# openpsi-project/srl

Measured on NVIDIA B200. Metric: gae_ppo_loss_transitions_per_sec, higher is better.
Workload: dtype f32

## Files before the change

### include/srl_b200.h

```cpp
#ifndef SRL_B200_H_
#define SRL_B200_H_

#include <stddef.h>
#include <stdint.h>

#ifdef __cplusplus
extern "C" {
#endif

#define SRL_B200_ABI_VERSION 12

typedef void* srl_stream_t;

enum srl_status {
  SRL_OK = 0,
  SRL_ERR_INVALID_ARG = 1,
  SRL_ERR_UNSUPPORTED = 2,
  SRL_ERR_CUDA = 3,
  SRL_ERR_NO_DEVICE = 4
};

const char* srl_last_error(void);
int srl_abi_version(void);
int srl_pdl_enabled(void);
int srl_set_pdl(int on);
int srl_device_info(int* sm_count, int* cc_major, int* cc_minor);

#define SRL_LANE_PART 8

int srl_gae_scan(const float* reward,
                 const float* value,
                 const uint8_t* done,
                 const uint8_t* truncated,
                 const uint8_t* on_reset,
                 const float* vtrace_new_logp,
                 const float* vtrace_old_logp,
                 const double* popart_mean_std,
                 const float* old_logp,
                 int L, int N, int row_lo, int row_hi, double gamma, double lmbda, double rho, double c,
                 float* adv,
                 float* ret,
                 double* lane_part,
                 double* lane_aos,
                 float* pack,
                 srl_stream_t stream);

int srl_gae_scan_perm(const float* reward, const float* value, const uint8_t* done, const uint8_t* truncated,
                      const uint8_t* on_reset, const float* vtrace_new_logp, const float* vtrace_old_logp,
                      const double* popart_mean_std, const float* old_logp, int L, int N, int row_lo, int row_hi,
                      double gamma, double lmbda, double rho, double c, float* adv, float* ret, double* lane_part,
                      double* lane_aos, float* pack, uint64_t perm_seed, uint32_t perm_epoch, int perm_n_epochs,
                      int perm_n_env, int perm_group, int32_t* perm_out, int perm_minibatches, double* minibatch_part,
                      int* fused, srl_stream_t stream);

int srl_gae_trace(const float* reward,
                  const float* value,
                  const uint8_t* done,
                  const uint8_t* truncated,
                  const uint8_t* on_reset,
                  const float* gamma_t,
                  const float* lmbda_t,
                  const float* imp_ratio,
                  int L, int N, int critic_dim, double gamma, double lmbda, double rho, double c, int pad_last_row,
                  float* adv, float* ret, srl_stream_t stream);

int srl_traj_gae(const void* reward, const void* value, const int64_t* offsets ,
                 const uint8_t* final_truncated ,
                 const uint8_t* final_has_value , int n_traj, int width, int is_float64,
                 double gamma, double lmbda, void* adv, void* ret, srl_stream_t stream);

int srl_n_step_return(const float* reward, const float* nex_value, const uint8_t* nex_done,
                      const uint8_t* nex_truncated, int n, int rows, int N, double gamma, float* out,
                      srl_stream_t stream);

int srl_lane_stats(const float* adv, const float* ret, const uint8_t* done, const uint8_t* truncated,
                   const uint8_t* on_reset, int L, int N, int row_lo, int row_hi, double* lane_part,
                   srl_stream_t stream);

size_t srl_group_stats_workspace_bytes(int G, int whole_first);
int srl_group_stats(const double* lane_part, int N, const int32_t* idx, int G, int per, int whole_first,
                    double* out, void* workspace, size_t workspace_bytes, srl_stream_t stream);

int srl_popart_update(const double* batch_stats, double* state, double beta, double eps, double* mean_std_out,
                      srl_stream_t stream);

enum srl_value_loss { SRL_VL_MSE = 0, SRL_VL_HUBER = 1, SRL_VL_SMOOTHL1 = 2 };

// ... 184 lines not shown
```

### srl_b200/_lib.py

```python
from __future__ import annotations

import ctypes
import os
from ctypes import POINTER, c_char_p, c_double, c_int, c_int32, c_int64, c_size_t, c_uint32, c_uint64, c_void_p

_HERE = os.path.dirname(os.path.abspath(__file__))
_LIB_NAME = "libsrl_b200.so"

SRL_LANE_PART = 8
SRL_LOSS_OUT_LEN = 16
SRL_MAX_LEAVES = 32
SRL_MAX_HEADS = 8
SRL_K4B_MAX_SUM_K = 199
SRL_K4B_MAX_SUM_K_MASKED = 159
SRL_MAX_LOSS_BATCH = 32
ABI_VERSION = 12

OUT_LOSS, OUT_POLICY_LOSS, OUT_VALUE_LOSS, OUT_ENTROPY_LOSS = 0, 1, 2, 3
OUT_ADVANTAGE, OUT_IMPORTANCE_WEIGHT, OUT_CLIP_RATIO, OUT_VALUE_TARGETS, OUT_DENORM_VALUE, OUT_MASK_SUM = 4, 5, 6, 7, 8, 9
VALUE_LOSS_CODES = {"mse": 0, "huber": 1, "smoothl1": 2}


class MissingCudaLibrary(RuntimeError):
    """libsrl_b200.so has not been built; run `python -m srl_b200.build` (needs nvcc)."""


class SrlCudaError(RuntimeError):

    def __init__(self, fn: str, status: int, message: str):
        super().__init__(f"{fn} failed with status {status}: {message}")
        self.fn, self.status, self.message = fn, status, message


class PpoHyper(ctypes.Structure):
    _fields_ = [
        ("eps_clip", c_double),
        ("value_eps_clip", c_double),
        ("c_clip", c_double),
        ("value_loss_weight", c_double),
        ("entropy_bonus_weight", c_double),
        ("vl_param", c_double),
        ("adv_eps", c_double),
        ("value_loss", c_int32),
        ("clip_value", c_int32),
        ("dual_clip", c_int32),
        ("normalize_old_value", c_int32),
    ]


class LossProblem(ctypes.Structure):
    _fields_ = [(k, c_void_p) for k in ("new_logp", "v_pred", "entropy", "lane_idx", "norm_stats", "local_stats",
                                        "g_logp", "g_value", "g_entropy", "out", "out_f32", "workspace")]


class LeafDesc(ctypes.Structure):
    _fields_ = [("src", c_void_p), ("dst", c_void_p), ("row_bytes", c_int64), ("src_slots", c_int64),
                ("src_t_stride", c_int64), ("src_slot_stride", c_int64)]


SIGNATURES = {
    "srl_last_error": (c_char_p, []),
    "srl_abi_version": (c_int, []),
    "srl_pdl_enabled": (c_int, []),
    "srl_set_pdl": (c_int, [c_int]),
    "srl_device_info": (c_int, [POINTER(c_int), POINTER(c_int), POINTER(c_int)]),
    "srl_gae_scan": (c_int, [c_void_p] * 9 + [c_int, c_int, c_int, c_int, c_double, c_double, c_double, c_double] +
                     [c_void_p, c_void_p, c_void_p, c_void_p, c_void_p, c_void_p]),
    "srl_gae_scan_perm": (c_int, [c_void_p] * 9 + [c_int, c_int, c_int, c_int, c_double, c_double, c_double, c_double] +
                          [c_void_p, c_void_p, c_void_p, c_void_p, c_void_p] +
                          [ctypes.c_uint64, ctypes.c_uint32, c_int, c_int, c_int, c_void_p, c_int, c_void_p, c_void_p,
                           c_void_p]),
    "srl_gae_trace": (c_int, [c_void_p] * 8 + [c_int, c_int, c_int, c_double, c_double, c_double, c_double, c_int,
                              c_void_p, c_void_p, c_void_p]),
    "srl_traj_gae": (c_int, [c_void_p] * 5 + [c_int, c_int, c_int, c_double, c_double, c_void_p, c_void_p, c_void_p]),
    "srl_n_step_return": (c_int, [c_void_p] * 4 + [c_int, c_int, c_int, c_double, c_void_p, c_void_p]),
    "srl_lane_stats": (c_int, [c_void_p] * 5 + [c_int, c_int, c_int, c_int, c_void_p, c_void_p]),
    "srl_group_stats_workspace_bytes": (c_size_t, [c_int, c_int]),
    "srl_group_stats": (c_int, [c_void_p, c_int, c_void_p, c_int, c_int, c_int, c_void_p, c_void_p, c_size_t, c_void_p]),
    "srl_popart_update": (c_int, [c_void_p, c_void_p, c_double, c_double, c_void_p, c_void_p]),
    "srl_ppo_loss_workspace_bytes": (c_size_t, [c_int, c_int]),
    "srl_ppo_loss_finalize": (c_int, [c_void_p, c_size_t, c_int, c_void_p, c_void_p, c_void_p]),
    "srl_ppo_loss_fwd_bwd": (c_int, [c_void_p, c_void_p, c_void_p, c_int64,
                                     c_void_p, c_void_p, c_void_p, c_void_p, c_void_p, c_int64, c_void_p,
                                     c_int, c_int, c_void_p, c_void_p, c_void_p, POINTER(PpoHyper),
                                     c_void_p, c_void_p, c_void_p, c_int64, c_void_p, c_void_p, c_void_p, c_size_t,
                                     c_void_p]),
    "srl_ppo_loss_fwd_bwd_batched": (c_int, [POINTER(LossProblem), c_int, c_int64, c_int64,
                                             c_void_p, c_void_p, c_void_p, c_void_p, c_void_p, c_int64, c_void_p,
                                             c_int, c_void_p, c_void_p, c_int, c_int, c_int, c_int, c_void_p, POINTER(PpoHyper),
                                             c_size_t, c_void_p, c_void_p]),
    "srl_ppo_loss_from_logits": (c_int, [c_void_p, c_void_p, POINTER(c_int32), c_int, c_void_p,
                                         c_void_p, c_void_p, c_void_p, c_void_p, c_void_p, c_int64, c_void_p,
                                         c_int, c_int, c_void_p, c_void_p, c_void_p, POINTER(PpoHyper),
                                         c_void_p, c_void_p, c_void_p, c_void_p, c_void_p, c_void_p, c_void_p,
                                         c_size_t, c_void_p]),
    "srl_ppo_loss_from_logits_masked": (c_int, [c_void_p, c_void_p, c_void_p, POINTER(c_int32), c_int, c_void_p,
                                                c_void_p, c_void_p, c_void_p, c_void_p, c_void_p, c_int64, c_void_p,
                                                c_int, c_int, c_void_p, c_void_p, c_void_p, POINTER(PpoHyper),
                                                c_void_p, c_void_p, c_void_p, c_void_p, c_void_p, c_void_p, c_void_p,
                                                c_size_t, c_void_p]),
    "srl_ppo_loss_from_logits_bf16": (c_int, [c_void_p, c_void_p, POINTER(c_int32), c_int, c_void_p,
                                              c_void_p, c_void_p, c_void_p, c_void_p, c_void_p, c_int64, c_void_p,
                                              c_int, c_int, c_void_p, c_void_p, c_void_p, POINTER(PpoHyper),
                                              c_void_p, c_void_p, c_void_p, c_void_p, c_void_p, c_void_p, c_void_p,
# ... 106 lines not shown
```

### srl_b200/csrc/gae_common.cuh

```cuda
#pragma once
#include <cuda_runtime.h>
#include <stdint.h>

#include "perm.cuh"

namespace srl {

struct GaeParams {
  const float* reward;
  const float* value;
  const uint8_t* done;
  const uint8_t* truncated;
  const uint8_t* on_reset;
  const float* vt_new_logp;
  const float* vt_old_logp;
  const double* popart;
  const float* old_logp;
  float* adv;
  float* ret;
  double* lane_part;
  double* lane_aos;
  float* pack;
  int L, N, row_lo, row_hi;
  double gamma, gamma_lmbda, rho, c;
  PermJob perm;
};

__host__ __device__ inline size_t pack_index(int t, int N, int lane) {
  return (static_cast<size_t>(t >> 1) * N + lane) * 2 + (t & 1);
}
constexpr int kPackMaskedAdv = 0x7fc00000;

bool gae_tma_eligible(const GaeParams& p);
int launch_gae_tma(const GaeParams& p, cudaStream_t st);
bool gae_ws_eligible(const GaeParams& p);
int launch_gae_ws(const GaeParams& p, cudaStream_t st);

#ifdef __CUDACC__

__device__ __forceinline__ float gae_vprime(float value, bool done, bool popart, double pa_mean, double pa_std) {
  if (popart) value = static_cast<float>(__dadd_rn(__dmul_rn(static_cast<double>(value), pa_std), pa_mean));
  return __fmul_rn(value, done ? 0.f : 1.f);
}

template <class V, class R>
__device__ __forceinline__ double gae_delta(const R* reward, V v0, V v1, bool reset1, double gamma) {
  double d = __dmul_rn(__dmul_rn(gamma, static_cast<double>(v1)), reset1 ? 0.0 : 1.0);
  d = __dadd_rn(static_cast<double>(*reward), d);
  return __dsub_rn(d, static_cast<double>(v0));
}

__device__ __forceinline__ double gae_carry_product(double gl, bool reset1, bool trunc1) {
  return __dmul_rn(__dmul_rn(gl, reset1 ? 0.0 : 1.0), trunc1 ? 0.0 : 1.0);
}
__device__ __forceinline__ double gae_carry(bool carries, double gl) { return carries ? gl : 0.0; }

__device__ __forceinline__ void gae_vtrace_scale(double& d, double& m, double ratio, double rho, double c) {
  d = __dmul_rn(d, fmin(ratio, rho));
// ... 46 lines not shown
```

### srl_b200/csrc/gae_scan.cu

```cuda
#include <stdlib.h>

#include "common.cuh"
#include "gae_common.cuh"

namespace srl {
namespace {

constexpr int kThreads = 256;
constexpr size_t kSmemBudget = 200 * 1024;

__host__ __device__ constexpr size_t gae_smem_bytes(int L, int LW, bool pack) {
  const size_t tile = static_cast<size_t>(L) * LW * (16 + 4 + 4 + 1 + (pack ? 8 : 0));
  const size_t scratch = static_cast<size_t>(kThreads) * 7 * 8;
  return tile > scratch ? tile : scratch;
}

template <int LW, bool VTRACE, bool PACK, int UN>
__global__ void __launch_bounds__(kThreads, 4) gae_scan_kernel(const GaeParams p) {
  constexpr int kUnroll = UN;
  constexpr int RPP = kThreads / LW;
  extern __shared__ __align__(16) unsigned char smem_raw[];
  const int L = p.L, N = p.N;
  const size_t cells = static_cast<size_t>(L) * LW;
  double2* __restrict__ sdm = reinterpret_cast<double2*>(smem_raw);
// ... 171 lines not shown

template <int LW, bool VTRACE, bool PACK, int UN>
int launch_un(const GaeParams& p, cudaStream_t st) {
  const size_t smem = gae_smem_bytes(p.L, LW, PACK);
  constexpr auto kern = gae_scan_kernel<LW, VTRACE, PACK, UN>;
  const int rc = opt_in_smem<kern>(kSmemBudget);
  if (rc != SRL_OK) return rc;
  const int grid = (p.N + LW - 1) / LW;
  SRL_CUDA(launch_pdl_scan(kern, dim3(grid), dim3(kThreads), smem, st, p));
  return SRL_OK;
}

template <int LW, bool VTRACE>
int launch(const GaeParams& p, cudaStream_t st) {
  constexpr int RPP = kThreads / LW;
  const int rows_per_thread = (p.L + RPP - 1) / RPP;
  if (!VTRACE && rows_per_thread == 5)
    return p.pack != nullptr ? launch_un<LW, false, true, 5>(p, st) : launch_un<LW, false, false, 5>(p, st);
  if (!VTRACE && rows_per_thread == 6)
    return p.pack != nullptr ? launch_un<LW, false, true, 6>(p, st) : launch_un<LW, false, false, 6>(p, st);
  if (p.pack != nullptr) return launch_un<LW, VTRACE, true, 4>(p, st);
  return launch_un<LW, VTRACE, false, 4>(p, st);
}

}
}

namespace srl {
namespace {
int gae_scan_impl(const float* reward, const float* value, const uint8_t* done, const uint8_t* truncated,
                  const uint8_t* on_reset, const float* vtrace_new_logp, const float* vtrace_old_logp,
                  const double* popart_mean_std, const float* old_logp, int L, int N, int row_lo, int row_hi, double gamma,
                  double lmbda, double rho, double c, float* adv, float* ret, double* lane_part, double* lane_aos, float* pack,
                  const PermJob* job, int* fused, srl_stream_t stream);
}
}

extern "C" int srl_gae_scan(const float* reward, const float* value, const uint8_t* done, const uint8_t* truncated,
                            const uint8_t* on_reset, const float* vtrace_new_logp, const float* vtrace_old_logp,
                            const double* popart_mean_std, const float* old_logp, int L, int N, int row_lo,
                            int row_hi, double gamma, double lmbda, double rho, double c, float* adv, float* ret,
                            double* lane_part, double* lane_aos, float* pack, srl_stream_t stream) {
  return srl::gae_scan_impl(reward, value, done, truncated, on_reset, vtrace_new_logp, vtrace_old_logp, popart_mean_std,
                            old_logp, L, N, row_lo, row_hi, gamma, lmbda, rho, c, adv, ret, lane_part, lane_aos, pack, nullptr,
                            nullptr, stream);
}

extern "C" int srl_gae_scan_perm(const float* reward, const float* value, const uint8_t* done, const uint8_t* truncated,
                                 const uint8_t* on_reset, const float* vtrace_new_logp, const float* vtrace_old_logp,
                                 const double* popart_mean_std, const float* old_logp, int L, int N, int row_lo,
                                 int row_hi, double gamma, double lmbda, double rho, double c, float* adv, float* ret,
                                 double* lane_part, double* lane_aos, float* pack, uint64_t perm_seed, uint32_t perm_epoch,
                                 int perm_n_epochs, int perm_n_env, int perm_group, int32_t* perm_out,
                                 int perm_minibatches, double* minibatch_part, int* fused, srl_stream_t stream) {
  using namespace srl;
  SRL_REQUIRE(perm_out != nullptr && perm_n_env >= 1 && perm_group >= 1 && perm_n_epochs >= 1 && perm_n_epochs <= 65535,
              SRL_ERR_INVALID_ARG, "srl_gae_scan_perm: need a permutation output, n_env >= 1, group >= 1, 1 <= n_epochs <= 65535");
  SRL_REQUIRE(static_cast<long long>(perm_n_env) * perm_group < (1ll << 31), SRL_ERR_UNSUPPORTED,
              "srl_gae_scan_perm: n_env * group must fit int32");
  PermJob job;
  job.seed_lo = static_cast<uint32_t>(perm_seed & 0xffffffffull);
  job.seed_hi = static_cast<uint32_t>(perm_seed >> 32);
  job.epoch0 = perm_epoch;
  job.n_epochs = perm_n_epochs;
  job.n_env = perm_n_env;
  job.group = perm_group;
  job.bits = perm_bits(perm_n_env);
  job.out = perm_out;
  job.minibatches = 1;
  job.per_mb = perm_n_env * perm_group;
  job.part = nullptr;
  if (minibatch_part != nullptr) {
    SRL_REQUIRE(perm_minibatches >= 1 && (static_cast<long long>(perm_n_env) * perm_group) % perm_minibatches == 0 &&
                    perm_n_env * perm_group == N && lane_part != nullptr && aligned(minibatch_part, 32),
                SRL_ERR_INVALID_ARG,
                "srl_gae_scan_perm: minibatch_part needs lane_part, n_env * group == N lanes split evenly into the minibatches "
                "and a 32-byte aligned table");
    if (perm_n_epochs <= kPartEpochs && perm_n_epochs * perm_minibatches <= kPartSlots) {
      job.minibatches = perm_minibatches;
      job.per_mb = perm_n_env * perm_group / perm_minibatches;
      job.part = minibatch_part;
    }
  }
  int did = 0;
  const int rc = gae_scan_impl(reward, value, done, truncated, on_reset, vtrace_new_logp, vtrace_old_logp, popart_mean_std,
                               old_logp, L, N, row_lo, row_hi, gamma, lmbda, rho, c, adv, ret, lane_part, lane_aos, pack, &job,
                               &did, stream);
  if (rc != SRL_OK) return rc;
  if (fused != nullptr) *fused = did ? (job.part != nullptr ? 2 : 1) : 0;
  if (did) return SRL_OK;
  return srl_philox_perm(perm_seed, perm_epoch, perm_n_epochs, perm_n_env, perm_group, perm_out, stream);
}

namespace srl {
namespace {
int gae_scan_impl(const float* reward, const float* value, const uint8_t* done, const uint8_t* truncated,
                  const uint8_t* on_reset, const float* vtrace_new_logp, const float* vtrace_old_logp,
                  const double* popart_mean_std, const float* old_logp, int L, int N, int row_lo, int row_hi, double gamma,
                  double lmbda, double rho, double c, float* adv, float* ret, double* lane_part, double* lane_aos, float* pack,
                  const PermJob* job, int* fused, srl_stream_t stream) {

  SRL_REQUIRE(L >= 2 && N >= 1, SRL_ERR_INVALID_ARG, "srl_gae_scan: need L >= 2 and N >= 1 (got L=%d N=%d)", L, N);
  SRL_REQUIRE(reward && value && done && truncated && on_reset && adv && ret, SRL_ERR_INVALID_ARG,
              "srl_gae_scan: null tensor pointer");
  SRL_REQUIRE((vtrace_new_logp == nullptr) == (vtrace_old_logp == nullptr), SRL_ERR_INVALID_ARG,
              "srl_gae_scan: vtrace needs both log-prob tensors");
  SRL_REQUIRE(row_lo >= 0 && row_lo <= row_hi && row_hi <= L - 1, SRL_ERR_INVALID_ARG,
              "srl_gae_scan: loss rows [%d, %d) must lie inside [0, L-1=%d]", row_lo, row_hi, L - 1);
  SRL_REQUIRE(pack == nullptr || (old_logp != nullptr && aligned(pack, 32)), SRL_ERR_INVALID_ARG,
              "srl_gae_scan: the pack needs old_logp and a 32-byte aligned destination");
  SRL_REQUIRE(lane_aos == nullptr || (lane_part != nullptr && aligned(lane_aos, 32)), SRL_ERR_INVALID_ARG,
              "srl_gae_scan: lane_aos needs lane_part and a 32-byte aligned destination");
  const bool vtrace = vtrace_new_logp != nullptr;
  GaeParams p;
  p.reward = reward;
  p.value = value;
  p.done = done;
  p.truncated = truncated;
  p.on_reset = on_reset;
  p.vt_new_logp = vtrace_new_logp;
  p.vt_old_logp = vtrace_old_logp;
  p.popart = popart_mean_std;
  p.old_logp = old_logp;
  p.pack = pack;
  p.adv = adv;
  p.ret = ret;
  p.lane_part = lane_part;
  p.lane_aos = lane_aos;
  p.L = L;
  p.N = N;
  p.row_lo = row_lo;
  p.row_hi = row_hi;
  p.gamma = gamma;
  p.gamma_lmbda = gamma * lmbda;
  p.rho = rho;
  p.c = c;
  p.perm.out = nullptr;
  p.perm.part = nullptr;
  cudaStream_t st = static_cast<cudaStream_t>(stream);

  const int groups = (N + 31) / 32;
  if (groups >= 2 * sm_count() && gae_tma_eligible(p)) return launch_gae_tma(p, st);
  if (groups >= 8 && gae_ws_eligible(p)) {
    if (job != nullptr) {
      p.perm = *job;
      *fused = 1;
    }
    return launch_gae_ws(p, st);
  }

  const int sms = sm_count();
  int lw = 32;
  const bool with_pack = pack != nullptr;
  while (lw > 8 && (gae_smem_bytes(L, lw, with_pack) > kSmemBudget || (N + lw - 1) / lw < 2 * sms)) lw >>= 1;
#ifdef SRL_DEBUG_PHASES
  if (const char* e = getenv("SRL_GAE_LW")) lw = atoi(e);
#endif
  SRL_REQUIRE(gae_smem_bytes(L, lw, with_pack) <= kSmemBudget, SRL_ERR_UNSUPPORTED,
              "srl_gae_scan: L=%d does not fit the shared-memory tile (max L ~ %d)", L,
              static_cast<int>(kSmemBudget / (8 * 25)));
  if (vtrace) {
    if (lw == 32) return launch<32, true>(p, st);
    if (lw == 16) return launch<16, true>(p, st);
    return launch<8, true>(p, st);
  }
  if (lw == 32) return launch<32, false>(p, st);
  if (lw == 16) return launch<16, false>(p, st);
  return launch<8, false>(p, st);
}
}
}
// ... 1 lines not shown
```

### srl_b200/csrc/gae_scan_ws.cu

```cuda
#include "gae_common.cuh"
#include "tma_util.cuh"

namespace srl {
namespace {

using namespace srl::tma;

__device__ __forceinline__ void st_cg256(float4* p, float4 a, float4 b) {
  asm volatile("st.global.cg.v8.f32 [%0], {%1, %2, %3, %4, %5, %6, %7, %8};" ::"l"(p), "f"(a.x), "f"(a.y), "f"(a.z), "f"(a.w),
               "f"(b.x), "f"(b.y), "f"(b.z), "f"(b.w)
               : "memory");
}

constexpr int kR = 16;
constexpr int kDeep = 9;

struct alignas(64) WsMaps {
  CUtensorMap value, reward, done, truncated, on_reset, old_logp;
};
struct WsParams {
  GaeParams p;
  WsMaps maps;
};

template <bool PACK>
struct Slot {
  static constexpr int value = 0;
  static constexpr int reward = value + (kR + 1) * 128;
  static constexpr int old_logp = reward + kR * 128;
  static constexpr int done = old_logp + (PACK ? kR * 128 : 0);
  static constexpr int truncated = done + 640;
  static constexpr int on_reset = truncated + 640;
  static constexpr int tx_bytes = (kR + 1) * 128 + kR * 128 + (PACK ? kR * 128 : 0) + 3 * (kR + 1) * 32;
  static constexpr int delta = on_reset + 640;
  static constexpr int mflag = delta + kR * 256;
  static constexpr int adv = mflag + kR * 32;
  static constexpr int vprime = adv + kR * 128;
  static constexpr int bytes = vprime + kR * 128;
  static_assert(bytes % 128 == 0, "slots stay 128-byte aligned");
};

template <int kS>
struct Bars {
  uint64_t tma_full[kS], pass1[kS], scanned[kS], empty[kS];
// ... 21 lines not shown
  if (threadIdx.x == 0) {
    for (int s = 0; s < kS; ++s) {
      mbar_init(&bars->tma_full[s], 1);
      mbar_init(&bars->pass1[s], kW);
      mbar_init(&bars->scanned[s], 1);
      mbar_init(&bars->empty[s], kW);
    }
    mbar_fence_init();
  }
  __syncthreads();
  if (threadIdx.x == 0) SRL_TL(1, blockIdx.x, 1);

  if (warp == 0) {
    if (lane == 0) {
      prefetch_map(&q.maps.value);
      prefetch_map(&q.maps.reward);
      prefetch_map(&q.maps.done);
      prefetch_map(&q.maps.truncated);
      prefetch_map(&q.maps.on_reset);
      for (int c = 0; c < n_chunks; ++c) {
        const int s = c % kS;
        if (c >= kS) mbar_wait(&bars->empty[s], ((c / kS) - 1) & 1);
        unsigned char* slot = smem + s * SL::bytes;
        const int row0 = (n_chunks - 1 - c) * kR;
        mbar_expect_tx(&bars->tma_full[s], SL::tx_bytes);
        tma_load_2d(slot + SL::value, &q.maps.value, col0, row0, &bars->tma_full[s]);
        tma_load_2d(slot + SL::reward, &q.maps.reward, col0, row0, &bars->tma_full[s]);
        tma_load_2d(slot + SL::done, &q.maps.done, col0, row0, &bars->tma_full[s]);
        tma_load_2d(slot + SL::truncated, &q.maps.truncated, col0, row0, &bars->tma_full[s]);
        tma_load_2d(slot + SL::on_reset, &q.maps.on_reset, col0, row0, &bars->tma_full[s]);
        if (PACK) tma_load_2d(slot + SL::old_logp, &q.maps.old_logp, col0, row0, &bars->tma_full[s]);
      }
      SRL_TL(1, blockIdx.x, 2);
    }
  } else if (warp == 1) {
    const double gl = p.gamma_lmbda;
    double g = 0.0;
    for (int c = 0; c < n_chunks; ++c) {
      const int s = c % kS;
      unsigned char* slot = smem + s * SL::bytes;
      mbar_wait(&bars->pass1[s], (c / kS) & 1);
      const double* sd = reinterpret_cast<const double*>(slot + SL::delta);
      const uint8_t* sm = slot + SL::mflag;
      float* sa = reinterpret_cast<float*>(slot + SL::adv);
      double d[kR];
      double m[kR];
#pragma unroll
      for (int r = 0; r < kR; ++r) {
        d[r] = sd[r * 32 + lane];
        m[r] = gae_carry(sm[r * 32 + lane] != 0, gl);
      }
#pragma unroll
      for (int r = kR - 1; r >= 0; --r) {
        g = gae_step(d[r], m[r], g);
        sa[r * 32 + lane] = static_cast<float>(g);
      }
      __syncwarp();
      if (lane == 0) mbar_arrive(&bars->scanned[s]);
    }
    if (lane == 0) SRL_TL(1, blockIdx.x, 4);
  } else {
    const int w = warp - 2;
    const bool popart = p.popart != nullptr;
    double pa_mean = 0.0, pa_std = 1.0;
    if (popart) {
      pa_mean = p.popart[0];
// ... 196 lines not shown
```

### srl_b200/hotpath.py

```python
from __future__ import annotations

import os
from typing import Dict, List, Optional

import numpy as np
import torch

from srl_b200 import ops
from srl_b200._lib import SRL_LANE_PART, SRL_LOSS_OUT_LEN

SAMPLE_F32 = ("reward", "value", "old_logp")
SAMPLE_U8 = ("done", "truncated", "on_reset")


def exchange_stats(local: torch.Tensor, out: torch.Tensor, group=None) -> torch.Tensor:
    out.copy_(local)
    torch.distributed.all_reduce(out, op=torch.distributed.ReduceOp.SUM, group=group)
    return out


class HotPath:

    def __init__(self, L: int, B: int, A: int = 1, *, gamma: float, lmbda: float, hyper: ops.LossHyper,
                 bootstrap_steps: int = 1, burn_in_steps: int = 0, epochs: int = 1, minibatches: int = 1, seed: int = 0,
# ... 97 lines not shown
        if t is None or t.numel() != like.size or t.dtype != torch.from_numpy(like.reshape(-1)[:1]).dtype:
            t = torch.empty(like.size, dtype=torch.from_numpy(like.reshape(-1)[:1]).dtype).pin_memory()
            self._pin[key] = t
        return t

    def load_sample(self, sample: Dict[str, np.ndarray], non_blocking: bool = True) -> int:
        moved = 0
        for k in SAMPLE_F32 + SAMPLE_U8:
            x = sample[k]
            want = np.float32 if k in SAMPLE_F32 else np.uint8
            if isinstance(x, torch.Tensor) and x.is_cuda:
                if x.numel() != self.L * self.N:
                    raise ValueError(f"{k}: {tuple(x.shape)} does not hold L*N = {self.L}*{self.N} elements")
                self.leaf[k].view(-1).copy_(x.reshape(-1), non_blocking=True)
                continue
            if isinstance(x, torch.Tensor):
                if x.is_pinned() and x.dtype == (torch.float32 if k in SAMPLE_F32 else torch.uint8) and \
                        x.numel() == self.L * self.N and x.is_contiguous():
                    self.leaf[k].view(-1).copy_(x.view(-1), non_blocking=non_blocking)
                    moved += x.numel() * x.element_size()
                    continue
                x = x.numpy()
            if x.size != self.L * self.N:
                raise ValueError(f"{k}: {x.shape} does not hold L*N = {self.L}*{self.N} elements")
            if x.dtype != want:
                x = x.astype(want)
            pin = self._pinned(k, x)
            pin.numpy()[:] = x.reshape(-1)
            self.leaf[k].view(-1).copy_(pin, non_blocking=non_blocking)
            moved += x.nbytes
        return moved

    def advantages(self, cached: bool = False, vtrace_new_logp: Optional[torch.Tensor] = None,
                   permute: bool = True) -> None:
        lf = self.leaf
        main = torch.cuda.current_stream()
        inline_perm = self.minibatches > 1 and permute and ops.pdl_enabled() and not cached
        fork_perm = self.minibatches > 1 and permute and not inline_perm
        perm_first = inline_perm and os.environ.get("SRL_PERM_FIRST") == "1"
        if perm_first:
            self.permute()
        if fork_perm:
            self._perm_stream.wait_stream(main)
            with torch.cuda.stream(self._perm_stream):
                self.permute()
        self.pack_valid = False
        job = None
        if cached:
            ops.lane_stats(self.adv, self.ret, lf["done"], lf["truncated"], lf["on_reset"], self.row_lo, self.row_hi,
                           lane_part=self.lane_part)
        else:
            kw = {}
            if vtrace_new_logp is not None:
                kw = dict(vtrace_new_logp=vtrace_new_logp, vtrace_old_logp=lf["old_logp"])
            elif self.pack is not None:
                kw = dict(old_logp=lf["old_logp"], pack=self.pack, lane_aos=self.lane_aos)
                self.pack_valid = True
            if inline_perm and not perm_first and os.environ.get("SRL_PERM_FUSED", "1") != "0":
                job = self.perm_job(with_part="lane_aos" in kw)
                kw["perm_job"] = job
            ops.gae_scan(lf["reward"], lf["value"], lf["done"], lf["truncated"], lf["on_reset"], self.gamma, self.lmbda,
                         row_lo=self.row_lo, row_hi=self.row_hi, popart_mean_std=self.popart_mean_std(), adv=self.adv,
                         ret=self.ret, lane_part=self.lane_part, **kw)
            self._perm_fused = bool(job and job.get("fused"))
        self._part_valid = bool(job and job.get("part_valid"))
        if inline_perm and not perm_first and job is None:
            self.permute()
        if fork_perm:
            main.wait_stream(self._perm_stream)
        self._lazy_table = self.fuse_stats and not cached
        self._stats_pending = self._lazy_table
        self._table_valid = False
        if not self._lazy_table:
            self.ensure_table()

    def perm_job(self, with_part: bool = True) -> dict:
        blk = self.shuffle_block
        job = dict(seed=self.seed + self.step_count, epoch=0, n_epochs=self.epochs, n_env=self.B // blk,
                   group=self.A * blk, out=self.perm)
        if self.mb_part is not None and with_part:
            job.update(minibatches=self.minibatches, part=self.mb_part)
        return job

    def ensure_table(self) -> None:
        if self._table_valid:
            return
        xk = dict(exchange=self.peer, global_out=self.global_stats) if (self.peer is not None and self.pg is not None) else {}
        if self.minibatches > 1:
            ops.group_stats(self.lane_part, idx=self.perm.view(-1), groups=self.epochs * self.minibatches,
                            per=self.n_mb, out=self.local_stats, whole_first=True, workspace=self.stats_ws, **xk)
        else:
            ops.group_stats(self.lane_part, groups=1, per=self.N, out=self.local_stats[0:1], workspace=self.stats_ws,
                            **xk)
# ... 106 lines not shown
            for e in range(self.epochs):
                if self.popart:
                    self.update_popart()
                for j in range(self.minibatches):
                    self.loss(e, j, *pol[e][j])
        elif self.popart:
            used = self._side[:min(branches, self.minibatches)]
            for e in range(self.epochs):
                self.update_popart()
                for st in used:
                    st.wait_stream(main)
                for j in range(self.minibatches):
                    with torch.cuda.stream(used[j % len(used)]):
                        self.loss(e, j, *pol[e][j])
                for st in used:
                    main.wait_stream(st)
        else:
            used = self._side[:min(branches, self.epochs * self.minibatches)]
            for st in used:
                st.wait_stream(main)
            for k in range(self.epochs * self.minibatches):
                e, j = divmod(k, self.minibatches)
                with torch.cuda.stream(used[k % len(used)]):
                    self.loss(e, j, *pol[e][j])
            for st in used:
                main.wait_stream(st)
        self.finalize()

    def run_device(self, pol, use_graph: bool = True, plan: bool = False) -> None:
        if plan:
            self._run_plan(pol)
            return
        if not use_graph:
            self.advantages()
            self._run_losses(pol)
            self.step_count += 1
            return
        if self._graph is None or self._graph_pol is not pol:
            self._capture(pol)
        if self._graph_a is None:
            self._graph.replay()
        else:
            self._graph_a.replay()
            self.exchange()
            self._graph.replay()
        self._table_valid = not self._lazy_table
        self.step_count += 1

    def plan_supported(self) -> bool:
        return (self.pg is None or self.peer is not None) and self._immediate and \
            (self.minibatches == 1 or ops.pdl_enabled())

    def _run_plan(self, pol) -> None:
        from srl_b200 import _lib
        st = torch.cuda.current_stream().cuda_stream
        if getattr(self, "_plan", None) is None or self._plan_pol is not pol or self._plan_stream != st:
            if not self.plan_supported():
                raise RuntimeError("HotPath.run_device(plan=True): the step holds launches that are not this library's (a "
                                   "torch.distributed exchange, side streams); use the CUDA graph")
            saved, self.step_count = self.step_count, 0
            calls = []
            try:
                with _lib.record_calls(calls):
                    self.advantages()
                    self._run_losses(pol)
            finally:
                self.step_count = saved
            self._plan, self._plan_pol, self._plan_stream = _lib.bind_calls(calls), pol, st
            self.plan_launch_calls = len(calls)
        else:
            _lib.replay_calls(self._plan)
            self._table_valid = not self._lazy_table
        self.step_count += 1

    def run_trainer_order(self, pol, use_graph: bool = True) -> None:
        if not use_graph:
            self._trainer_order_launches(pol)
            self.step_count += 1
            return
        if getattr(self, "_graph_to", None) is None or self._graph_to_pol is not pol:
            saved = self.step_count
            self.step_count = 0
            s = torch.cuda.Stream()
            s.wait_stream(torch.cuda.current_stream())
            with torch.cuda.stream(s):
                self._trainer_order_launches(pol)
            torch.cuda.current_stream().wait_stream(s)
            torch.cuda.synchronize()
            g = torch.cuda.CUDAGraph()
            with torch.cuda.graph(g):
                self._trainer_order_launches(pol)
            self._graph_to, self._graph_to_pol = g, pol
            self.step_count = saved
        self._graph_to.replay()
        self.step_count += 1

    def _trainer_order_launches(self, pol) -> None:
        self.advantages()
        self._join_stats()
        for e in range(self.epochs):
            if self.popart:
                self.update_popart()
            for j in range(self.minibatches):
                self.loss(e, j, *pol[e][j])
        self.finalize()

    def loss_chain_graph(self, pol) -> torch.cuda.CUDAGraph:
        def chain():
            for e in range(self.epochs):
                for j in range(self.minibatches):
                    self.loss(e, j, *pol[e][j])
        s = torch.cuda.Stream()
        s.wait_stream(torch.cuda.current_stream())
        with torch.cuda.stream(s):
            chain()
        torch.cuda.current_stream().wait_stream(s)
        torch.cuda.synchronize()
        g = torch.cuda.CUDAGraph()
        with torch.cuda.graph(g):
            chain()
        return g

    def _capture(self, pol) -> None:
        saved = self.step_count
        self.step_count = 0
        s = torch.cuda.Stream()
        s.wait_stream(torch.cuda.current_stream())
        with torch.cuda.stream(s):
            self.advantages()
            self._run_losses(pol)
        torch.cuda.current_stream().wait_stream(s)
        torch.cuda.synchronize()
        self._graph_a = None
        if self.pg is None or self.peer is not None:
            g = torch.cuda.CUDAGraph()
            with torch.cuda.graph(g):
                self.advantages()
                self._run_losses(pol, self.graph_branches)
            self._graph = g
        else:
            pg, self.pg = self.pg, None
            try:
                ga, gb = torch.cuda.CUDAGraph(), torch.cuda.CUDAGraph()
                with torch.cuda.graph(ga):
                    self.advantages()
                with torch.cuda.graph(gb):
                    self._run_losses(pol, self.graph_branches)
                self._graph_a, self._graph = ga, gb
            finally:
                self.pg = pg
        self.step_count = saved
        self._graph_pol = pol
        self.launches_per_step = self.count_launches()

    def count_launches(self) -> int:
        n = 1 if self.fuse_stats else 2
        if self.minibatches > 1 and not self._perm_fused:
            n += 1
        if self._immediate:
            per_launch = 32
            if self.popart:
                n += self.epochs * (1 + -(-self.minibatches // per_launch))
            else:
                n += -(-(self.epochs * self.minibatches) // per_launch)
            return n
        per_loss = 1 if (self.fuse_gather or self.minibatches == 1) else 2
        n += self.epochs * self.minibatches * per_loss
        n += 1
        if self.popart:
            n += self.epochs
        return n

    def run_host(self, sample: Dict[str, np.ndarray], pol_host: torch.Tensor, out_host: Dict[str, torch.Tensor],
                 use_graph: bool = True, pol_device: Optional[torch.Tensor] = None) -> Dict[str, int]:
        E, Mb = self.epochs, self.minibatches
        if not hasattr(self, "_pol_dev_all"):
            self._pol_dev_all = torch.empty((E, Mb, 3, self.T, self.n_mb), dtype=torch.float32, device=self.device)
            self._pol_dev = [[tuple(self._pol_dev_all[e, j, q] for q in range(3)) for j in range(Mb)] for e in range(E)]
# ... 131 lines not shown
```

### srl_b200/ops.py

```python
from __future__ import annotations

import ctypes
import dataclasses
from typing import List, Optional, Sequence, Tuple

import torch

from srl_b200 import _lib
from srl_b200._lib import (SRL_LANE_PART, SRL_LOSS_OUT_LEN, SRL_MAX_HEADS, SRL_MAX_LEAVES, SRL_MAX_LOSS_BATCH, LeafDesc, LossProblem,
                           PpoHyper, VALUE_LOSS_CODES)


def _stream() -> int:
    return torch.cuda.current_stream().cuda_stream


def _ptr(t: Optional[torch.Tensor]) -> Optional[int]:
    return None if t is None else t.data_ptr()


def _check(t: torch.Tensor, dtype, name: str) -> torch.Tensor:
    if not isinstance(t, torch.Tensor) or not t.is_cuda:
        raise ValueError(f"{name}: expected a CUDA tensor (srl_b200 has no CPU path), got {type(t).__name__}"
                         f"{'' if not isinstance(t, torch.Tensor) else ' on ' + str(t.device)}")
    if t.dtype != dtype:
        raise ValueError(f"{name}: expected dtype {dtype}, got {t.dtype}")
    if not t.is_contiguous():
        raise ValueError(f"{name}: expected a contiguous tensor, got strides {t.stride()} for shape {tuple(t.shape)}")
    return t


def _check_view(t: torch.Tensor, dtype, name: str) -> torch.Tensor:
    if not isinstance(t, torch.Tensor) or not t.is_cuda:
        raise ValueError(f"{name}: expected a CUDA tensor (srl_b200 has no CPU path)")
    if t.dtype != dtype:
        raise ValueError(f"{name}: expected dtype {dtype}, got {t.dtype}")
    return t


def _rows_lanes(t: torch.Tensor) -> Tuple[int, int]:
    if t.dim() < 2:
        raise ValueError(f"expected a time-major [L, N, ...] tensor, got shape {tuple(t.shape)}")
    return t.shape[0], t[0].numel()


def pdl_enabled() -> bool:
    return bool(_lib.load_library().srl_pdl_enabled())


def set_pdl(on: bool) -> bool:
    return bool(_lib.load_library().srl_set_pdl(int(bool(on))))


def gae_scan(reward, value, done, truncated, on_reset, gamma: float, lmbda: float, row_lo: int = 0,
             row_hi: Optional[int] = None, popart_mean_std: Optional[torch.Tensor] = None,
             vtrace_new_logp: Optional[torch.Tensor] = None, vtrace_old_logp: Optional[torch.Tensor] = None,
             rho: float = 1.0, c: float = 1.0, adv: Optional[torch.Tensor] = None,
             ret: Optional[torch.Tensor] = None, lane_part: Optional[torch.Tensor] = None, want_stats: bool = True,
             old_logp: Optional[torch.Tensor] = None, pack: Optional[torch.Tensor] = None,
             lane_aos: Optional[torch.Tensor] = None, perm_job: Optional[dict] = None):
    L, N = _rows_lanes(value)
    for name, t in (("reward", reward), ("value", value)):
        _check(t, torch.float32, name)
    for name, t in (("done", done), ("truncated", truncated), ("on_reset", on_reset)):
        _check(t, torch.uint8, name)
    for name, t in (("reward", reward), ("done", done), ("truncated", truncated), ("on_reset", on_reset)):
        if _rows_lanes(t) != (L, N):
            raise ValueError(f"{name}: shape {tuple(t.shape)} does not match value {tuple(value.shape)}")
    if row_hi is None:
        row_hi = L - 1
    if (vtrace_new_logp is None) != (vtrace_old_logp is None):
        raise ValueError("vtrace needs both new and old log-probs")
    for name, t in (("vtrace_new_logp", vtrace_new_logp), ("vtrace_old_logp", vtrace_old_logp)):
        if t is not None:
            _check(t, torch.float32, name)
            if t.shape[0] < L - 1 or t[0].numel() != N:
                raise ValueError(f"{name}: need at least L-1={L - 1} rows of {N} lanes, got {tuple(t.shape)}")
    if popart_mean_std is not None:
        _check(popart_mean_std, torch.float64, "popart_mean_std")
    adv = torch.empty_like(value) if adv is None else _check(adv, torch.float32, "adv")
    ret = torch.empty_like(value) if ret is None else _check(ret, torch.float32, "ret")
    if want_stats and lane_part is None:
        lane_part = torch.empty((SRL_LANE_PART, N), dtype=torch.float64, device=value.device)
    if lane_part is not None:
        _check(lane_part, torch.float64, "lane_part")
        if tuple(lane_part.shape) != (SRL_LANE_PART, N):
            raise ValueError(f"lane_part: expected shape {(SRL_LANE_PART, N)}, got {tuple(lane_part.shape)}")
    if pack is not None:
        _check(pack, torch.float32, "pack")
        if old_logp is None:
            raise ValueError("pack needs old_logp")
        _check(old_logp, torch.float32, "old_logp")
        if pack.numel() != pack_rows(L) * N * 4 or _rows_lanes(old_logp) != (L, N):
            raise ValueError(f"pack must hold [ceil(L/2), N, 2, 4] = {pack_rows(L) * N * 4} floats and old_logp [L, N]; got "
                             f"{tuple(pack.shape)} and {tuple(old_logp.shape)}")
    if lane_aos is not None:
        _check(lane_aos, torch.float64, "lane_aos")
        if lane_part is None or tuple(lane_aos.shape) != (N, 4):
            raise ValueError(f"lane_aos needs lane_part and shape {(N, 4)}, got {tuple(lane_aos.shape)}")
    args = (_ptr(reward), _ptr(value), _ptr(done), _ptr(truncated), _ptr(on_reset),
            _ptr(vtrace_new_logp), _ptr(vtrace_old_logp), _ptr(popart_mean_std),
            _ptr(old_logp) if pack is not None else None, L, N, int(row_lo), int(row_hi),
            float(gamma), float(lmbda), float(rho), float(c), _ptr(adv), _ptr(ret), _ptr(lane_part), _ptr(lane_aos),
            _ptr(pack))
    if perm_job is None:
        _lib.call("srl_gae_scan", *args, _stream())
    else:
        out = _check(perm_job["out"], torch.int32, "perm_job['out']")
        n_ep, n_env, group = int(perm_job["n_epochs"]), int(perm_job["n_env"]), int(perm_job.get("group", 1))
        if out.numel() != n_ep * n_env * group:
            raise ValueError(f"perm_job['out'] must hold [n_epochs, n_env * group] = {n_ep * n_env * group} int32")
        part = perm_job.get("part")
        if part is not None:
            _check(part, torch.float64, "perm_job['part']")
            if tuple(part.shape) != (SRL_MAX_LOSS_BATCH, (N + 31) // 32, 4):
                raise ValueError(f"perm_job['part']: expected new_minibatch_part(N) = {(SRL_MAX_LOSS_BATCH, (N + 31) // 32, 4)}, "
                                 f"got {tuple(part.shape)}")
        fused = ctypes.c_int(0)
        _lib.call("srl_gae_scan_perm", *args, ctypes.c_uint64(int(perm_job["seed"]) & (2 ** 64 - 1)),
                  ctypes.c_uint32(int(perm_job.get("epoch", 0))), n_ep, n_env, group, _ptr(out),
                  int(perm_job.get("minibatches", 1)), _ptr(part), ctypes.byref(fused), _stream())
        perm_job["fused"] = fused.value >= 1
        perm_job["part_valid"] = fused.value == 2
    return adv, ret, lane_part


def new_minibatch_part(N: int, device) -> torch.Tensor:
    return torch.zeros((SRL_MAX_LOSS_BATCH, (N + 31) // 32, 4), dtype=torch.float64, device=device)


def pack_rows(L: int) -> int:
    return L + (L & 1)


def new_pack(L: int, N: int, device) -> torch.Tensor:
    return torch.empty((pack_rows(L) // 2, N, 2, 4), dtype=torch.float32, device=device)


def unpack_rows(pack: torch.Tensor) -> torch.Tensor:
    P, N = pack.shape[0], pack.shape[1]
    return pack.permute(0, 2, 1, 3).reshape(2 * P, N, 4)


def gae_trace(reward, value, truncated, done, on_reset, gamma, lmbda, vtrace: bool = False, imp_ratio=None,
              rho: float = 1.0, c: float = 1.0, high_precision: bool = True, apply_done: bool = False,
              want_ret: bool = False, pad_last_row: bool = False):
    if not high_precision:
        raise NotImplementedError("gae_trace: only the float64 scan (high_precision=True, the reference's default)")
    for name, t in (("reward", reward), ("value", value)):
        _check(t, torch.float32, name)
    for name, t in (("truncated", truncated), ("done", done), ("on_reset", on_reset)):
        _check(t, torch.uint8, name)
    L = value.shape[0]
    if L < 2 or reward.shape[0] < L - 1:
        raise ValueError(f"value needs >= 2 rows and reward >= L-1 rows; got {tuple(value.shape)}, {tuple(reward.shape)}")
    N = on_reset[0].numel()
    if value[0].numel() % N != 0:
# ... 723 lines not shown
```

Before: 17.46 billion.

## Prefetch policy loss tensors into L2 from the GAE scan producer warp

Adds a warm variant of the fused GAE scan plus permutation entry point that takes up to eight device address ranges. Once the producer warp has issued its last TMA load, it spreads these ranges across blocks and issues bulk L2 prefetches, so the loss kernel that follows finds its policy inputs already in L2. The hot path passes the policy tensors as warm ranges. The risk is extra DRAM traffic competing with the scan, and L2 thrashing if the ranges exceed cache capacity; ranges beyond the first eight merged spans are dropped silently.

Result: no change. 17.60 billion (median of 6 runs) (+0.8%).

```diff
diff --git a/include/srl_b200.h b/include/srl_b200.h
--- a/include/srl_b200.h
+++ b/include/srl_b200.h
@@ -53,6 +53,16 @@
                       int perm_n_env, int perm_group, int32_t* perm_out, int perm_minibatches, double* minibatch_part,
                       int* fused, srl_stream_t stream);
 
+#define SRL_MAX_L2_WARM 8
+int srl_gae_scan_perm_warm(const float* reward, const float* value, const uint8_t* done, const uint8_t* truncated,
+                           const uint8_t* on_reset, const float* vtrace_new_logp, const float* vtrace_old_logp,
+                           const double* popart_mean_std, const float* old_logp, int L, int N, int row_lo, int row_hi,
+                           double gamma, double lmbda, double rho, double c, float* adv, float* ret, double* lane_part,
+                           double* lane_aos, float* pack, uint64_t perm_seed, uint32_t perm_epoch, int perm_n_epochs,
+                           int perm_n_env, int perm_group, int32_t* perm_out, int perm_minibatches, double* minibatch_part,
+                           const void* const* warm_ptr, const uint64_t* warm_bytes, int n_warm, int* fused,
+                           srl_stream_t stream);
+
 int srl_gae_trace(const float* reward,
                   const float* value,
                   const uint8_t* done,
diff --git a/srl_b200/_lib.py b/srl_b200/_lib.py
--- a/srl_b200/_lib.py
+++ b/srl_b200/_lib.py
@@ -14,6 +14,7 @@
 SRL_K4B_MAX_SUM_K = 199
 SRL_K4B_MAX_SUM_K_MASKED = 159
 SRL_MAX_LOSS_BATCH = 32
+SRL_MAX_L2_WARM = 8
 ABI_VERSION = 12
 
 OUT_LOSS, OUT_POLICY_LOSS, OUT_VALUE_LOSS, OUT_ENTROPY_LOSS = 0, 1, 2, 3
@@ -70,6 +71,10 @@
                           [c_void_p, c_void_p, c_void_p, c_void_p, c_void_p] +
                           [ctypes.c_uint64, ctypes.c_uint32, c_int, c_int, c_int, c_void_p, c_int, c_void_p, c_void_p,
                            c_void_p]),
+    "srl_gae_scan_perm_warm": (c_int, [c_void_p] * 9 + [c_int, c_int, c_int, c_int, c_double, c_double, c_double, c_double] +
+                               [c_void_p, c_void_p, c_void_p, c_void_p, c_void_p] +
+                               [ctypes.c_uint64, ctypes.c_uint32, c_int, c_int, c_int, c_void_p, c_int, c_void_p,
+                                POINTER(c_void_p), POINTER(ctypes.c_uint64), c_int, c_void_p, c_void_p]),
     "srl_gae_trace": (c_int, [c_void_p] * 8 + [c_int, c_int, c_int, c_double, c_double, c_double, c_double, c_int,
                               c_void_p, c_void_p, c_void_p]),
     "srl_traj_gae": (c_int, [c_void_p] * 5 + [c_int, c_int, c_int, c_double, c_double, c_void_p, c_void_p, c_void_p]),
diff --git a/srl_b200/csrc/gae_common.cuh b/srl_b200/csrc/gae_common.cuh
--- a/srl_b200/csrc/gae_common.cuh
+++ b/srl_b200/csrc/gae_common.cuh
@@ -5,6 +5,13 @@
 #include "perm.cuh"
 
 namespace srl {
+
+constexpr int kMaxL2Warm = SRL_MAX_L2_WARM;
+struct L2Warm {
+  const char* ptr[kMaxL2Warm];
+  unsigned long long bytes[kMaxL2Warm];
+  int n;
+};
 
 struct GaeParams {
   const float* reward;
@@ -24,6 +31,7 @@
   int L, N, row_lo, row_hi;
   double gamma, gamma_lmbda, rho, c;
   PermJob perm;
+  L2Warm warm;
 };
 
 __host__ __device__ inline size_t pack_index(int t, int N, int lane) {
diff --git a/srl_b200/csrc/gae_scan.cu b/srl_b200/csrc/gae_scan.cu
--- a/srl_b200/csrc/gae_scan.cu
+++ b/srl_b200/csrc/gae_scan.cu
@@ -227,7 +227,7 @@
                   const uint8_t* on_reset, const float* vtrace_new_logp, const float* vtrace_old_logp,
                   const double* popart_mean_std, const float* old_logp, int L, int N, int row_lo, int row_hi, double gamma,
                   double lmbda, double rho, double c, float* adv, float* ret, double* lane_part, double* lane_aos, float* pack,
-                  const PermJob* job, int* fused, srl_stream_t stream);
+                  const PermJob* job, const L2Warm* warm, int* fused, srl_stream_t stream);
 }
 }
 
@@ -238,17 +238,18 @@
                             double* lane_part, double* lane_aos, float* pack, srl_stream_t stream) {
   return srl::gae_scan_impl(reward, value, done, truncated, on_reset, vtrace_new_logp, vtrace_old_logp, popart_mean_std,
                             old_logp, L, N, row_lo, row_hi, gamma, lmbda, rho, c, adv, ret, lane_part, lane_aos, pack, nullptr,
-                            nullptr, stream);
-}
-
-extern "C" int srl_gae_scan_perm(const float* reward, const float* value, const uint8_t* done, const uint8_t* truncated,
-                                 const uint8_t* on_reset, const float* vtrace_new_logp, const float* vtrace_old_logp,
-                                 const double* popart_mean_std, const float* old_logp, int L, int N, int row_lo,
-                                 int row_hi, double gamma, double lmbda, double rho, double c, float* adv, float* ret,
-                                 double* lane_part, double* lane_aos, float* pack, uint64_t perm_seed, uint32_t perm_epoch,
-                                 int perm_n_epochs, int perm_n_env, int perm_group, int32_t* perm_out,
-                                 int perm_minibatches, double* minibatch_part, int* fused, srl_stream_t stream) {
-  using namespace srl;
+                            nullptr, nullptr, stream);
+}
+
+namespace srl {
+namespace {
+int gae_scan_perm_impl(const float* reward, const float* value, const uint8_t* done, const uint8_t* truncated,
+                       const uint8_t* on_reset, const float* vtrace_new_logp, const float* vtrace_old_logp,
+                       const double* popart_mean_std, const float* old_logp, int L, int N, int row_lo, int row_hi,
+                       double gamma, double lmbda, double rho, double c, float* adv, float* ret, double* lane_part,
+                       double* lane_aos, float* pack, uint64_t perm_seed, uint32_t perm_epoch, int perm_n_epochs,
+                       int perm_n_env, int perm_group, int32_t* perm_out, int perm_minibatches, double* minibatch_part,
+                       const L2Warm* warm, int* fused, srl_stream_t stream) {
   SRL_REQUIRE(perm_out != nullptr && perm_n_env >= 1 && perm_group >= 1 && perm_n_epochs >= 1 && perm_n_epochs <= 65535,
               SRL_ERR_INVALID_ARG, "srl_gae_scan_perm: need a permutation output, n_env >= 1, group >= 1, 1 <= n_epochs <= 65535");
   SRL_REQUIRE(static_cast<long long>(perm_n_env) * perm_group < (1ll << 31), SRL_ERR_UNSUPPORTED,
@@ -280,11 +281,53 @@
   int did = 0;
   const int rc = gae_scan_impl(reward, value, done, truncated, on_reset, vtrace_new_logp, vtrace_old_logp, popart_mean_std,
                                old_logp, L, N, row_lo, row_hi, gamma, lmbda, rho, c, adv, ret, lane_part, lane_aos, pack, &job,
-                               &did, stream);
+                               warm, &did, stream);
   if (rc != SRL_OK) return rc;
   if (fused != nullptr) *fused = did ? (job.part != nullptr ? 2 : 1) : 0;
   if (did) return SRL_OK;
   return srl_philox_perm(perm_seed, perm_epoch, perm_n_epochs, perm_n_env, perm_group, perm_out, stream);
+}
+}
+}
+
+extern "C" int srl_gae_scan_perm(const float* reward, const float* value, const uint8_t* done, const uint8_t* truncated,
+                                 const uint8_t* on_reset, const float* vtrace_new_logp, const float* vtrace_old_logp,
+                                 const double* popart_mean_std, const float* old_logp, int L, int N, int row_lo,
+                                 int row_hi, double gamma, double lmbda, double rho, double c, float* adv, float* ret,
+                                 double* lane_part, double* lane_aos, float* pack, uint64_t perm_seed, uint32_t perm_epoch,
+                                 int perm_n_epochs, int perm_n_env, int perm_group, int32_t* perm_out,
+                                 int perm_minibatches, double* minibatch_part, int* fused, srl_stream_t stream) {
+  return srl::gae_scan_perm_impl(reward, value, done, truncated, on_reset, vtrace_new_logp, vtrace_old_logp,
+                                 popart_mean_std, old_logp, L, N, row_lo, row_hi, gamma, lmbda, rho, c, adv, ret, lane_part,
+                                 lane_aos, pack, perm_seed, perm_epoch, perm_n_epochs, perm_n_env, perm_group, perm_out,
+                                 perm_minibatches, minibatch_part, nullptr, fused, stream);
+}
+
+extern "C" int srl_gae_scan_perm_warm(const float* reward, const float* value, const uint8_t* done,
+                                      const uint8_t* truncated, const uint8_t* on_reset, const float* vtrace_new_logp,
+                                      const float* vtrace_old_logp, const double* popart_mean_std, const float* old_logp,
+                                      int L, int N, int row_lo, int row_hi, double gamma, double lmbda, double rho, double c,
+                                      float* adv, float* ret, double* lane_part, double* lane_aos, float* pack,
+                                      uint64_t perm_seed, uint32_t perm_epoch, int perm_n_epochs, int perm_n_env,
+                                      int perm_group, int32_t* perm_out, int perm_minibatches, double* minibatch_part,
+                                      const void* const* warm_ptr, const uint64_t* warm_bytes, int n_warm, int* fused,
+                                      srl_stream_t stream) {
+  using namespace srl;
+  SRL_REQUIRE(n_warm >= 0 && n_warm <= SRL_MAX_L2_WARM && (n_warm == 0 || (warm_ptr != nullptr && warm_bytes != nullptr)),
+              SRL_ERR_INVALID_ARG, "srl_gae_scan_perm_warm: 0 <= n_warm <= %d ranges, host arrays of pointers and sizes",
+              SRL_MAX_L2_WARM);
+  L2Warm warm;
+  warm.n = n_warm;
+  for (int i = 0; i < n_warm; ++i) {
+    SRL_REQUIRE(warm_ptr[i] != nullptr || warm_bytes[i] == 0, SRL_ERR_INVALID_ARG,
+                "srl_gae_scan_perm_warm: range %d has no address", i);
+    warm.ptr[i] = static_cast<const char*>(warm_ptr[i]);
+    warm.bytes[i] = warm_bytes[i];
+  }
+  return gae_scan_perm_impl(reward, value, done, truncated, on_reset, vtrace_new_logp, vtrace_old_logp, popart_mean_std,
+                            old_logp, L, N, row_lo, row_hi, gamma, lmbda, rho, c, adv, ret, lane_part, lane_aos, pack,
+                            perm_seed, perm_epoch, perm_n_epochs, perm_n_env, perm_group, perm_out, perm_minibatches,
+                            minibatch_part, &warm, fused, stream);
 }
 
 namespace srl {
@@ -293,7 +336,7 @@
                   const uint8_t* on_reset, const float* vtrace_new_logp, const float* vtrace_old_logp,
                   const double* popart_mean_std, const float* old_logp, int L, int N, int row_lo, int row_hi, double gamma,
                   double lmbda, double rho, double c, float* adv, float* ret, double* lane_part, double* lane_aos, float* pack,
-                  const PermJob* job, int* fused, srl_stream_t stream) {
+                  const PermJob* job, const L2Warm* warm, int* fused, srl_stream_t stream) {
 
   SRL_REQUIRE(L >= 2 && N >= 1, SRL_ERR_INVALID_ARG, "srl_gae_scan: need L >= 2 and N >= 1 (got L=%d N=%d)", L, N);
   SRL_REQUIRE(reward && value && done && truncated && on_reset && adv && ret, SRL_ERR_INVALID_ARG,
@@ -332,6 +375,8 @@
   p.c = c;
   p.perm.out = nullptr;
   p.perm.part = nullptr;
+  p.warm.n = 0;
+  if (warm != nullptr) p.warm = *warm;
   cudaStream_t st = static_cast<cudaStream_t>(stream);
 
   const int groups = (N + 31) / 32;
diff --git a/srl_b200/csrc/gae_scan_ws.cu b/srl_b200/csrc/gae_scan_ws.cu
--- a/srl_b200/csrc/gae_scan_ws.cu
+++ b/srl_b200/csrc/gae_scan_ws.cu
@@ -10,6 +10,26 @@
   asm volatile("st.global.cg.v8.f32 [%0], {%1, %2, %3, %4, %5, %6, %7, %8};" ::"l"(p), "f"(a.x), "f"(a.y), "f"(a.z), "f"(a.w),
                "f"(b.x), "f"(b.y), "f"(b.z), "f"(b.w)
                : "memory");
+}
+
+__device__ __forceinline__ void warm_l2_share(const L2Warm& w) {
+  unsigned long long total = 0;
+  for (int i = 0; i < w.n; ++i) total += w.bytes[i];
+  const unsigned long long lo = total * blockIdx.x / gridDim.x & ~127ull;
+  const unsigned long long hi = blockIdx.x + 1 == gridDim.x ? total : (total * (blockIdx.x + 1) / gridDim.x & ~127ull);
+  unsigned long long base = 0;
+  for (int i = 0; i < w.n; ++i) {
+    const unsigned long long a = lo > base ? lo : base, b = hi < base + w.bytes[i] ? hi : base + w.bytes[i];
+    if (a < b) {
+      const unsigned long long s = (reinterpret_cast<unsigned long long>(w.ptr[i] + (a - base)) + 15) & ~15ull;
+      const unsigned long long e = reinterpret_cast<unsigned long long>(w.ptr[i] + (b - base)) & ~15ull;
+      for (unsigned long long q = s; q < e; q += 65536) {
+        const unsigned int len = static_cast<unsigned int>(e - q < 65536 ? e - q : 65536);
+        asm volatile("cp.async.bulk.prefetch.L2.global [%0], %1;" ::"l"(q), "r"(len) : "memory");
+      }
+    }
+    base += w.bytes[i];
+  }
 }
 
 constexpr int kR = 16;
@@ -97,6 +117,11 @@
         if (PACK) tma_load_2d(slot + SL::old_logp, &q.maps.old_logp, col0, row0, &bars->tma_full[s]);
       }
       SRL_TL(1, blockIdx.x, 2);
+      if (p.warm.n > 0) {
+        const int c = n_chunks - 1;
+        mbar_wait(&bars->tma_full[c % kS], (c / kS) & 1);
+        warm_l2_share(p.warm);
+      }
     }
   } else if (warp == 1) {
     const double gl = p.gamma_lmbda;
diff --git a/srl_b200/hotpath.py b/srl_b200/hotpath.py
--- a/srl_b200/hotpath.py
+++ b/srl_b200/hotpath.py
@@ -153,7 +153,7 @@
         return moved
 
     def advantages(self, cached: bool = False, vtrace_new_logp: Optional[torch.Tensor] = None,
-                   permute: bool = True) -> None:
+                   permute: bool = True, warm_pol=None) -> None:
         lf = self.leaf
         main = torch.cuda.current_stream()
         inline_perm = self.minibatches > 1 and permute and ops.pdl_enabled() and not cached
@@ -180,6 +180,8 @@
             if inline_perm and not perm_first and os.environ.get("SRL_PERM_FUSED", "1") != "0":
                 job = self.perm_job(with_part="lane_aos" in kw)
                 kw["perm_job"] = job
+                if warm_pol is not None:
+                    kw["l2_warm"] = [t for row in warm_pol for trio in row for t in trio]
             ops.gae_scan(lf["reward"], lf["value"], lf["done"], lf["truncated"], lf["on_reset"], self.gamma, self.lmbda,
                          row_lo=self.row_lo, row_hi=self.row_hi, popart_mean_std=self.popart_mean_std(), adv=self.adv,
                          ret=self.ret, lane_part=self.lane_part, **kw)
@@ -352,7 +354,7 @@
             self._run_plan(pol)
             return
         if not use_graph:
-            self.advantages()
+            self.advantages(warm_pol=pol)
             self._run_losses(pol)
             self.step_count += 1
             return
@@ -382,7 +384,7 @@
             calls = []
             try:
                 with _lib.record_calls(calls):
-                    self.advantages()
+                    self.advantages(warm_pol=pol)
                     self._run_losses(pol)
             finally:
                 self.step_count = saved
@@ -447,7 +449,7 @@
         s = torch.cuda.Stream()
         s.wait_stream(torch.cuda.current_stream())
         with torch.cuda.stream(s):
-            self.advantages()
+            self.advantages(warm_pol=pol)
             self._run_losses(pol)
         torch.cuda.current_stream().wait_stream(s)
         torch.cuda.synchronize()
@@ -455,7 +457,7 @@
         if self.pg is None or self.peer is not None:
             g = torch.cuda.CUDAGraph()
             with torch.cuda.graph(g):
-                self.advantages()
+                self.advantages(warm_pol=pol)
                 self._run_losses(pol, self.graph_branches)
             self._graph = g
         else:
@@ -463,7 +465,7 @@
             try:
                 ga, gb = torch.cuda.CUDAGraph(), torch.cuda.CUDAGraph()
                 with torch.cuda.graph(ga):
-                    self.advantages()
+                    self.advantages(warm_pol=pol)
                 with torch.cuda.graph(gb):
                     self._run_losses(pol, self.graph_branches)
                 self._graph_a, self._graph = ga, gb
diff --git a/srl_b200/ops.py b/srl_b200/ops.py
--- a/srl_b200/ops.py
+++ b/srl_b200/ops.py
@@ -7,8 +7,8 @@
 import torch
 
 from srl_b200 import _lib
-from srl_b200._lib import (SRL_LANE_PART, SRL_LOSS_OUT_LEN, SRL_MAX_HEADS, SRL_MAX_LEAVES, SRL_MAX_LOSS_BATCH, LeafDesc, LossProblem,
-                           PpoHyper, VALUE_LOSS_CODES)
+from srl_b200._lib import (SRL_LANE_PART, SRL_LOSS_OUT_LEN, SRL_MAX_HEADS, SRL_MAX_L2_WARM, SRL_MAX_LEAVES,
+                           SRL_MAX_LOSS_BATCH, LeafDesc, LossProblem, PpoHyper, VALUE_LOSS_CODES)
 
 
 def _stream() -> int:
@@ -58,7 +58,8 @@
              rho: float = 1.0, c: float = 1.0, adv: Optional[torch.Tensor] = None,
              ret: Optional[torch.Tensor] = None, lane_part: Optional[torch.Tensor] = None, want_stats: bool = True,
              old_logp: Optional[torch.Tensor] = None, pack: Optional[torch.Tensor] = None,
-             lane_aos: Optional[torch.Tensor] = None, perm_job: Optional[dict] = None):
+             lane_aos: Optional[torch.Tensor] = None, perm_job: Optional[dict] = None,
+             l2_warm: Optional[Sequence[torch.Tensor]] = None):
     L, N = _rows_lanes(value)
     for name, t in (("reward", reward), ("value", value)):
         _check(t, torch.float32, name)
@@ -104,6 +105,8 @@
             float(gamma), float(lmbda), float(rho), float(c), _ptr(adv), _ptr(ret), _ptr(lane_part), _ptr(lane_aos),
             _ptr(pack))
     if perm_job is None:
+        if l2_warm:
+            raise ValueError("l2_warm needs a perm_job (srl_gae_scan_perm_warm)")
         _lib.call("srl_gae_scan", *args, _stream())
     else:
         out = _check(perm_job["out"], torch.int32, "perm_job['out']")
@@ -117,12 +120,37 @@
                 raise ValueError(f"perm_job['part']: expected new_minibatch_part(N) = {(SRL_MAX_LOSS_BATCH, (N + 31) // 32, 4)}, "
                                  f"got {tuple(part.shape)}")
         fused = ctypes.c_int(0)
-        _lib.call("srl_gae_scan_perm", *args, ctypes.c_uint64(int(perm_job["seed"]) & (2 ** 64 - 1)),
-                  ctypes.c_uint32(int(perm_job.get("epoch", 0))), n_ep, n_env, group, _ptr(out),
-                  int(perm_job.get("minibatches", 1)), _ptr(part), ctypes.byref(fused), _stream())
+        job_args = (ctypes.c_uint64(int(perm_job["seed"]) & (2 ** 64 - 1)), ctypes.c_uint32(int(perm_job.get("epoch", 0))),
+                    n_ep, n_env, group, _ptr(out), int(perm_job.get("minibatches", 1)), _ptr(part))
+        if l2_warm:
+            ranges = l2_ranges(l2_warm)
+            ptrs = (ctypes.c_void_p * len(ranges))(*[a for a, _ in ranges])
+            sizes = (ctypes.c_uint64 * len(ranges))(*[n for _, n in ranges])
+            _lib.call("srl_gae_scan_perm_warm", *args, *job_args, ptrs, sizes, len(ranges), ctypes.byref(fused), _stream())
+        else:
+            _lib.call("srl_gae_scan_perm", *args, *job_args, ctypes.byref(fused), _stream())
         perm_job["fused"] = fused.value >= 1
         perm_job["part_valid"] = fused.value == 2
     return adv, ret, lane_part
+
+
+def l2_ranges(tensors: Sequence[torch.Tensor]) -> list:
+    spans = []
+    for t in tensors:
+        if not t.is_cuda:
+            raise ValueError("l2_warm: CUDA tensors only")
+        if t.numel() == 0:
+            continue
+        lo = t.data_ptr()
+        hi = lo + (sum((s - 1) * st for s, st in zip(t.shape, t.stride())) + 1) * t.element_size()
+        spans.append((lo, hi))
+    merged = []
+    for lo, hi in sorted(spans):
+        if merged and lo <= merged[-1][1]:
+            merged[-1][1] = max(merged[-1][1], hi)
+        else:
+            merged.append([lo, hi])
+    return [(lo, hi - lo) for lo, hi in merged[:SRL_MAX_L2_WARM]]
 
 
 def new_minibatch_part(N: int, device) -> torch.Tensor:
```
